# Adamtaranto/mimeo

Measured on NVIDIA B200. Metric: self-alignment Mbp/sec (genome Mbp annotated per second of hot-path time), higher is better.
Workload: dtype int32

## Files before the change

mimeo_b200/csrc/seed.cu:

```cuda
#include "primitives.cuh"
#include "seq.cuh"
#include "internal.cuh"
#include "xdrop_table.cuh"

namespace mb2 {

constexpr uint32_t KEY_INVALID = 1u << 24;
constexpr int S1_WINDOW = 30;
constexpr uint32_t S1_WINDOW_MASK = (1u << S1_WINDOW) - 1u;
constexpr int S1_RIGHT_WINDOWS = 2;
constexpr int S1_LEFT_WINDOWS = 3;
constexpr int S1_TAB = XT_SIZE;

__global__ void __launch_bounds__(256)
seed_keys_kernel(GenomeView T, uint32_t p_lo, uint32_t n, uint32_t* __restrict__ keys, uint32_t* __restrict__ pos) {
    const uint32_t k = blockIdx.x * blockDim.x + threadIdx.x;
    if (k >= n) return;
    const uint32_t p = p_lo + k;
    const uint32_t nw = nwindow32(T.sm, p) & SEED_WINDOW_MASK19;
    keys[k] = nw ? KEY_INVALID : seed_key(window32(T.pk, p));
    pos[k] = p;
}

__global__ void __launch_bounds__(256)
bucket_offsets_kernel(const uint32_t* __restrict__ keys, uint32_t n, uint32_t* __restrict__ off) {
    const uint32_t idx = blockIdx.x * blockDim.x + threadIdx.x;
    if (idx > n) return;
    const int64_t prev = idx == 0 ? -1 : (int64_t)keys[idx - 1];
    const int64_t cur = idx == n ? (int64_t)KEY_INVALID : (int64_t)min(keys[idx], KEY_INVALID);
    for (int64_t k = prev + 1; k <= cur; k++) off[k] = idx;
}

void build_seed_table(const Genome& T, uint32_t p_lo, uint32_t p_hi, SeedTable& tab) {
    const uint32_t n = p_hi - p_lo;
    ProfScope ps("seed_table_build");
    DevBuf<uint32_t> k0(n), k1(n), v0(n), v1(n);
    launch(seed_keys_kernel, cdiv(n, 256), 256, 0, view(T), p_lo, n, k0.get(), v0.get());
    const int w = radix_sort_bits<uint32_t, uint32_t>(k0.get(), k1.get(), v0.get(), v1.get(), n, 0, 25);
    tab.off.alloc((size_t)KEY_INVALID + 1);
    launch(bucket_offsets_kernel, cdiv((size_t)n + 1, 256), 256, 0, w ? k1.get() : k0.get(), n, tab.off.get());
    tab.pos = std::move(w ? v1 : v0);
    tab.p_lo = p_lo; tab.p_hi = p_hi;
}

constexpr int S1_DONE = 1 << 24;
constexpr int S1_D0 = 125;
constexpr int S1_MAX_XDROP = 8191 - 125 - 300;
__device__ __forceinline__ uint32_t s1_entry(uint32_t idx, int X) {
    const uint32_t q6 = idx >> 6, t6 = idx & 63;
    int sum = 0, mx = INT_MIN, mn = INT_MAX;
    for (int c = 0; c < 3; c++) {
        sum += sub_lut((((t6 >> (2 * c)) & 3u) << 2) | ((q6 >> (2 * c)) & 3u));
        mx = max(mx, sum); mn = min(mn, sum);
    }
    return ((uint32_t)sum << 22) | ((uint32_t)(mx + 125) << 13) | (uint32_t)(mn + X + 125);
}
__device__ __forceinline__ uint32_t s1_bits(uint32_t lo, uint32_t hi, int s) {
    return s <= 0 ? lo << (-s) : (s < 32 ? __funnelshift_r(lo, hi, s) : hi >> (s - 32));
}
template <uint32_t VOTES>
__device__ __forceinline__ void xdrop_window30(uint32_t tab_sa, uint32_t m10, uint32_t m9, uint64_t wt, uint64_t wq, uint32_t an, int X,
                                               int& best, int& D, uint32_t& nchunks) {
    int d_keep = 0;
    bool slow = false;
    if (D < S1_DONE / 2 && an) {
        int run = best - (D - 125);
        bool term = false;
        for (int c = 0; c < S1_WINDOW && !term; c++) {
            const int sc = (an & 1u) ? SCORE_N : sub_lut((uint32_t)((wt & 3) << 2 | (wq & 3)));
            wt >>= 2; wq >>= 2; an >>= 1;
            run += sc;
            if (run > best) best = run; else if (run < best - X) term = true;
        }
        nchunks += S1_WINDOW / 3;
        d_keep = term ? S1_DONE : (best - run) + 125;
        slow = true; D = S1_DONE;
    }
    const uint32_t tl = (uint32_t)wt, th = (uint32_t)(wt >> 32), ql = (uint32_t)wq, qh = (uint32_t)(wq >> 32);
    uint32_t parked = 0;
    int entered = S1_WINDOW / 3;
#pragma unroll
    for (int k = 0; k < S1_WINDOW / 3; k++) {
        if ((VOTES >> k) & 1u) { if (__all_sync(0xffffffffu, D >= S1_DONE / 2)) { entered = k; break; } }
        const uint32_t addr = ((s1_bits(tl, th, 6 * k - 2) & 0xFCu) | (s1_bits(ql, qh, 6 * k - 8) & 0x3F00u)) + tab_sa;
        uint32_t e;
        asm("ld.shared.u32 %0, [%1];" : "=r"(e) : "r"(addr));
        parked += (uint32_t)D;
        const bool term = (int)(e & 0x1FFFu) < D;
        const int dm = max(D, (int)__umulhi(e * m10, m9));
        best += dm - D;
        D = term ? S1_DONE : dm - __mulhi((int)e, (int)m10);
    }
    nchunks += (uint32_t)entered - (parked >> 24);
    if (slow) D = d_keep;
}
__device__ __forceinline__ uint32_t s1_pack(int best, int D) {
    return (uint32_t)best | ((D < S1_DONE / 2 ? (uint32_t)D : 0xFFFFu) << 16);
}
__device__ __forceinline__ void s1_unpack(uint32_t w, int& best, int& D) {
    best = (int)(w & 0xFFFFu);
    D = (w >> 16) == 0xFFFFu ? S1_DONE : (int)(w >> 16);
}

struct SeqBlock {
    uint64_t w[4];
    uint32_t n[4], s[4];
    uint32_t c0;
    __device__ __forceinline__ void windows(uint32_t p, uint64_t& f, uint64_t& l, uint64_t& r, uint32_t& fn, uint32_t& rn, uint32_t& ls) const {
        const uint32_t off = p - c0, sh = (off & 15u) * 2u;
        const bool b0 = off & 16u, b1 = off & 32u;
        uint32_t x[8], a[7], y[5];
#pragma unroll
        for (int m = 0; m < 4; m++) { x[2 * m] = (uint32_t)w[m]; x[2 * m + 1] = (uint32_t)(w[m] >> 32); }
#pragma unroll
        for (int m = 0; m < 7; m++) a[m] = b0 ? x[m + 1] : x[m];
#pragma unroll
        for (int m = 0; m < 5; m++) y[m] = b1 ? a[m + 2] : a[m];
        const uint32_t f0 = __funnelshift_r(y[0], y[1], sh), f1 = __funnelshift_r(y[1], y[2], sh);
        const uint32_t r0 = __funnelshift_r(y[2], y[3], sh), r1 = __funnelshift_r(y[3], y[4], sh);
        f = (uint64_t)f0 | ((uint64_t)f1 << 32); r = (uint64_t)r0 | ((uint64_t)r1 << 32);
        l = (uint64_t)__funnelshift_r(f0, f1, 24) | ((uint64_t)__funnelshift_r(f1, r0, 24) << 32);
        const uint32_t sn = off & 31u;
        const uint32_t n0 = b1 ? n[1] : n[0], n1 = b1 ? n[2] : n[1], n2 = b1 ? n[3] : n[2];
        fn = __funnelshift_r(n0, n1, sn); rn = __funnelshift_r(n1, n2, sn);
        const uint32_t s0 = b1 ? s[1] : s[0], s1 = b1 ? s[2] : s[1], s2 = b1 ? s[3] : s[2];
        ls = __funnelshift_r(__funnelshift_r(s0, s1, sn), __funnelshift_r(s1, s2, sn), 12);
    }
};
__device__ __forceinline__ SeqBlock load_block(const uint64_t* __restrict__ pk, const uint32_t* __restrict__ nm, const uint32_t* __restrict__ sm,
                                               uint32_t first) {
    SeqBlock b;
    b.c0 = first & ~63u;
    const uint32_t w0 = b.c0 >> 5;
    const uint4 a = *reinterpret_cast<const uint4*>(pk + w0), c = *reinterpret_cast<const uint4*>(pk + w0 + 2);
    b.w[0] = (uint64_t)a.x | ((uint64_t)a.y << 32); b.w[1] = (uint64_t)a.z | ((uint64_t)a.w << 32);
    b.w[2] = (uint64_t)c.x | ((uint64_t)c.y << 32); b.w[3] = (uint64_t)c.z | ((uint64_t)c.w << 32);
    const uint2 n0 = *reinterpret_cast<const uint2*>(nm + w0), n1 = *reinterpret_cast<const uint2*>(nm + w0 + 2);
    b.n[0] = n0.x; b.n[1] = n0.y; b.n[2] = n1.x; b.n[3] = n1.y;
    if (sm != nm) {
        const uint2 s0 = *reinterpret_cast<const uint2*>(sm + w0), s1 = *reinterpret_cast<const uint2*>(sm + w0 + 2);
        b.s[0] = s0.x; b.s[1] = s0.y; b.s[2] = s1.x; b.s[3] = s1.y;
    } else {
        b.s[0] = b.n[0]; b.s[1] = b.n[1]; b.s[2] = b.n[2]; b.s[3] = b.n[3];
    }
    return b;
}

__device__ __forceinline__ void append_survivors(bool survivor, uint32_t hi, uint32_t hj, uint32_t diag_bias, int lane,
                                                 uint64_t* __restrict__ surv, uint32_t surv_cap, unsigned long long* __restrict__ counters) {
    const uint32_t smask = __ballot_sync(0xffffffffu, survivor);
    if (smask) {
        unsigned long long basev = 0;
        if (lane == __ffs(smask) - 1) basev = atomicAdd(&counters[0], (unsigned long long)__popc(smask));
        basev = __shfl_sync(0xffffffffu, basev, __ffs(smask) - 1);
        if (survivor) {
            const unsigned long long slot = basev + __popc(smask & ((1u << lane) - 1u));
            if (slot < surv_cap) surv[slot] = ((uint64_t)(hi - hj + diag_bias) << 32) | hj;
        }
    }
}

constexpr int SC_NT = 256;
constexpr int SC_WARPS = SC_NT / 32;
constexpr int SC_NPROBE = 13;
constexpr int SC_HALF = 3;
constexpr int SC_STEPS = (SC_NPROBE + SC_HALF - 1) / SC_HALF;
constexpr int SC_RING = 128;
constexpr int SC_DQ = 64;

__device__ __forceinline__ void s1_later_window(const GenomeView& T, const GenomeView& Q, uint32_t hi, uint32_t hj, bool right, int b, int D,
                                                uint64_t& wt, uint64_t& wq, uint32_t& an) {
    wt = 0; wq = 0; an = 0;
    if (D >= S1_DONE / 2) return;
    if (right) {
        const uint32_t ct = hi + SEED_SPAN + S1_WINDOW * b, cq = hj + SEED_SPAN + S1_WINDOW * b;
        wt = window32(T.pk, ct); wq = window32(Q.pk, cq);
        an = (nwindow32(T.nm, ct) | nwindow32(Q.nm, cq)) & S1_WINDOW_MASK;
    } else {
        const uint32_t ct = hi + SEED_SPAN - S1_WINDOW * b - 32, cq = hj + SEED_SPAN - S1_WINDOW * b - 32;
        wt = rev2groups(window32(T.pk, ct)); wq = rev2groups(window32(Q.pk, cq));
        an = __brev(nwindow32(T.nm, ct) | nwindow32(Q.nm, cq)) & S1_WINDOW_MASK;
    }
}

template <int MINB, uint32_t TAILVOTES>
__global__ void __launch_bounds__(SC_NT, MINB)
seed_scan_kernel(GenomeView T, GenomeView Q, const uint32_t* __restrict__ off, const uint32_t* __restrict__ pos,
                 uint32_t q_lo, uint32_t q_n, int X, int K, int transition, uint32_t diag_bias,
                 uint64_t* __restrict__ surv, uint32_t surv_cap, unsigned long long* __restrict__ counters) {
    __shared__ uint32_t s1tab[S1_TAB];
    __shared__ uint32_t r_cum[SC_WARPS][SC_RING], r_b0[SC_WARPS][SC_RING], r_j[SC_WARPS][SC_RING];
    __shared__ uint4 r_defer[SC_WARPS][SC_DQ];
    __shared__ unsigned long long sh_stat[3];
    const int tid = threadIdx.x, lane = tid & 31, warp = tid >> 5;
    for (int e = tid; e < S1_TAB; e += SC_NT) s1tab[e] = s1_entry((uint32_t)e, X);
    const uint32_t s1tab_sa = (uint32_t)__cvta_generic_to_shared(s1tab);
    const uint32_t s1_m10 = q_n ? 1024u : 0u, s1_m9 = q_n ? 512u : 0u;
    if (tid < 3) sh_stat[tid] = 0;
    __syncthreads();
    uint32_t* __restrict__ rc = r_cum[warp];
    uint32_t* __restrict__ rb = r_b0[warp];
    uint32_t* __restrict__ rj = r_j[warp];
    uint4* __restrict__ dq = r_defer[warp];
    const int nprobe = transition ? SC_NPROBE : 1;
    const uint32_t nrounds = (q_n + 31) / 32;
    uint32_t round = 0;
    int part = SC_STEPS;
    bool exhausted = false;
    uint32_t head = 0, tail = 0;
    uint32_t cum_tail = 0, consumed = 0;
    uint32_t dq_head = 0, dq_tail = 0;
    unsigned long long n_lead = 0, n_cells = 0, n_hits = 0;
    for (;;) {
        while (cum_tail - consumed < 32u && !exhausted) {
            if (part == SC_STEPS) {
                unsigned long long r = 0;
                if (lane == 0) r = atomicAdd(&counters[CNT_WORK], 1ull);
                r = __shfl_sync(0xffffffffu, r, 0);
                if (r >= nrounds) { exhausted = true; break; }
                round = (uint32_t)r; part = 0;
            }
            const int p0 = part * SC_HALF, p1 = min(SC_NPROBE, p0 + SC_HALF);
            part++;
            const uint32_t jrel = round * 32 + lane;
            const uint32_t j = q_lo + jrel;
            const bool jvalid = jrel < q_n && (nwindow32(Q.sm, j) & SEED_WINDOW_MASK19) == 0;
            uint32_t key = 0;
            if (jvalid) key = seed_key(window32(Q.pk, j));
            uint32_t b0[SC_HALF], cnt[SC_HALF];
            uint32_t mine = 0, nne = 0;
#pragma unroll
            for (int q = 0; q < SC_HALF; q++) {
                const int pr = p0 + q;
                uint32_t c = 0, b = 0;
                if (jvalid && pr < p1 && pr < nprobe) {
                    const uint32_t kk = pr == 0 ? key : key ^ (2u << (2 * (pr - 1)));
                    b = off[kk];
                    c = off[kk + 1] - b;
                }
                b0[q] = b; cnt[q] = c;
                mine += c; nne += c ? 1u : 0u;
            }
            uint32_t sh = mine, sn = nne;
#pragma unroll
            for (int d = 1; d < 32; d <<= 1) {
                const uint32_t th = __shfl_up_sync(0xffffffffu, sh, d), tn = __shfl_up_sync(0xffffffffu, sn, d);
                if (lane >= d) { sh += th; sn += tn; }
            }
            const uint32_t tot_h = __shfl_sync(0xffffffffu, sh, 31), tot_n = __shfl_sync(0xffffffffu, sn, 31);
            uint32_t run = cum_tail + sh - mine, slot = tail + sn - nne;
#pragma unroll
            for (int q = 0; q < SC_HALF; q++) {
                if (cnt[q]) {
                    const uint32_t w = slot & (SC_RING - 1);
                    rc[w] = run; rb[w] = b0[q]; rj[w] = j;
                    run += cnt[q]; slot++;
                }
            }
            tail += tot_n; cum_tail += tot_h; n_hits += (lane == 0) ? tot_h : 0;
            __syncwarp();
        }
        const uint32_t pending = cum_tail - consumed, queued = dq_tail - dq_head;
        if (pending == 0 && queued == 0) break;
        uint32_t hi = 0, hj = 0, nchunks = 0;
        int best_r = 0, dr = S1_DONE, best_l = 0, dl = S1_DONE;
        bool live;
        if (queued >= 32u || pending == 0) {
            static_assert(S1_RIGHT_WINDOWS == 2 && S1_LEFT_WINDOWS == 3, "a batch runs right window 0 and left windows 0, 1; a drain the rest");
            const uint32_t nd = min(queued, 32u);
            live = (uint32_t)lane < nd;
            if (live) {
                const uint4 r = dq[(dq_head + (uint32_t)lane) & (SC_DQ - 1)];
                hi = r.x; hj = r.y;
                s1_unpack(r.z, best_r, dr);
                s1_unpack(r.w, best_l, dl);
            }
            dq_head += nd;
            uint64_t wt, wq; uint32_t an;
            if (!__all_sync(0xffffffffu, dr >= S1_DONE / 2)) {
                s1_later_window(T, Q, hi, hj, true, 1, dr, wt, wq, an);
                xdrop_window30<TAILVOTES>(s1tab_sa, s1_m10, s1_m9, wt, wq, an, X, best_r, dr, nchunks);
            }
            if (!__all_sync(0xffffffffu, dl >= S1_DONE / 2)) {
                s1_later_window(T, Q, hi, hj, false, 2, dl, wt, wq, an);
                xdrop_window30<TAILVOTES>(s1tab_sa, s1_m10, s1_m9, wt, wq, an, X, best_l, dl, nchunks);
            }
        } else {
            const uint32_t nb = min(pending, 32u);
            live = (uint32_t)lane < nb;
            const uint32_t h = consumed + (uint32_t)lane;
            uint32_t e_last = head;
            {
                const uint32_t di = head + (uint32_t)lane;
                const bool dv = (int32_t)(tail - di) > 0;
                const uint32_t ci = dv ? rc[di & (SC_RING - 1)] : 0u;
                const uint32_t first = ci - consumed;
                const uint32_t starts = __reduce_or_sync(0xffffffffu, (dv && lane > 0 && first < 32u) ? (1u << first) : 0u);
                if (live) {
                    const uint32_t lo = head + (uint32_t)__popc(starts & ((2u << lane) - 1u));
                    e_last = lo;
                    hi = pos[rb[lo & (SC_RING - 1)] + (h - rc[lo & (SC_RING - 1)])];
                    hj = rj[lo & (SC_RING - 1)];
                }
            }
            uint64_t lt = 0, lq = 0, rt = 0, rq = 0, ft = 0, fq = 0;
            uint32_t ln = 1, rn = 0, fn = 0;
            if (live) {
                const SeqBlock bt = load_block(T.pk, T.nm, T.sm, hi - 13), bq = load_block(Q.pk, Q.nm, Q.sm, hj - 13);
                uint32_t tfn, trn, tls, qfn, qrn, qls;
                bt.windows(hi - 13, ft, lt, rt, tfn, trn, tls);
                bq.windows(hj - 13, fq, lq, rq, qfn, qrn, qls);
                ln = (tls | qls) & SEED_WINDOW_MASK19;
                rn = (trn | qrn) & S1_WINDOW_MASK;
                fn = __brev(tfn | qfn) & S1_WINDOW_MASK;
                if (ln == 0 && seed_match(lt, lq, transition != 0)) live = false; else n_lead++;
            }
            if (live) { dr = S1_D0; dl = S1_D0; }
            xdrop_window30<0u>(s1tab_sa, s1_m10, s1_m9, rt, rq, rn, X, best_r, dr, nchunks);
            xdrop_window30<0u>(s1tab_sa, s1_m10, s1_m9, rev2groups(ft), rev2groups(fq), fn, X, best_l, dl, nchunks);
            if (!__all_sync(0xffffffffu, dl >= S1_DONE / 2)) {
                uint64_t wt, wq; uint32_t an;
                s1_later_window(T, Q, hi, hj, false, 1, dl, wt, wq, an);
                xdrop_window30<TAILVOTES>(s1tab_sa, s1_m10, s1_m9, wt, wq, an, X, best_l, dl, nchunks);
            }
            const bool defer = live && (dr < S1_DONE / 2 || dl < S1_DONE / 2);
            const uint32_t dmask = __ballot_sync(0xffffffffu, defer);
            if (defer) {
                dq[(dq_tail + (uint32_t)__popc(dmask & ((1u << lane) - 1u))) & (SC_DQ - 1)] =
                    make_uint4(hi, hj, s1_pack(best_r, dr), s1_pack(best_l, dl));
                live = false;
            }
            dq_tail += (uint32_t)__popc(dmask);
            consumed += nb;
            uint32_t e = __shfl_sync(0xffffffffu, e_last, (int)nb - 1);
            const uint32_t next_cum = (e + 1 < tail) ? rc[(e + 1) & (SC_RING - 1)] : cum_tail;
            head = ((int32_t)(next_cum - consumed) > 0) ? e : e + 1;
        }
        n_cells += 3ull * nchunks;
        append_survivors(live && (dr < S1_DONE / 2 || dl < S1_DONE / 2 || best_r + best_l >= K), hi, hj, diag_bias, lane, surv, surv_cap, counters);
        __syncwarp();
    }
    if (n_lead) atomicAdd(&sh_stat[1], n_lead);
    if (n_cells) atomicAdd(&sh_stat[2], n_cells);
    if (n_hits) atomicAdd(&sh_stat[0], n_hits);
    __syncthreads();
    if (tid < 3 && sh_stat[tid]) atomicAdd(&counters[1 + tid], sh_stat[tid]);
}

void seed_scan(const Genome& T, const Genome& Q, const SeedTable& tab, uint32_t q_lo, uint32_t q_hi, const AlignParams& p,
               uint64_t* surv, uint32_t surv_cap, unsigned long long* counters) {
    const uint32_t n = q_hi - q_lo;
    if (n == 0) return;
    MB2_REQUIRE(p.xdrop >= XT_MIN_XDROP, -2, "x-drop below 251 is not supported by the three-column extension table");
    MB2_REQUIRE(p.xdrop <= S1_MAX_XDROP, -2, "x-drop above 7766 is not supported by the first-stage extension table");
    ProfScope ps("seed_scan");
    const unsigned nrounds = cdiv(n, 32);
    static const int minb = getenv("MB2_SCAN_MINB") ? atoi(getenv("MB2_SCAN_MINB")) : 4;
    auto go = [&](auto kern) {
        int per_sm = 0;
        MB2_CUDA(cudaOccupancyMaxActiveBlocksPerMultiprocessor(&per_sm, kern, SC_NT, 0));
        const unsigned grid = std::min<unsigned>(cdiv(nrounds, SC_WARPS), (unsigned)ctx().sm_count * (unsigned)std::max(1, per_sm));
        launch(kern, grid, SC_NT, 0, view(T), view(Q), tab.off.get(), tab.pos.get(), q_lo, n, p.xdrop,
               p.hspthresh, p.transition, (uint32_t)Q.G, surv, surv_cap, counters);
    };
    if (minb <= 3) go(seed_scan_kernel<3, 0x148u>); else go(seed_scan_kernel<4, 0x148u>);
}

}
```

Baseline: 460.9.

## Extend seed block load to cover second left x-drop window from registers

The per-seed sequence block now loads one extra leading 64-bit packed word and N-mask word. This lets the second left-extension window be extracted by funnel shifts from registers instead of issuing separate global window loads in s1_later_window. The kernel's launch bounds are also replaced with explicit __maxnreg__ caps (56 or 80) to control register pressure from the larger block. It adds an unconditional extra load per live seed, even when the second left window is never needed, and reads at w0-1, which may fall before the buffer start near position zero.

```diff
diff --git a/mimeo_b200/csrc/seed.cu b/mimeo_b200/csrc/seed.cu
--- a/mimeo_b200/csrc/seed.cu
+++ b/mimeo_b200/csrc/seed.cu
@@ -103,26 +103,30 @@
 }
 
 struct SeqBlock {
-    uint64_t w[4];
-    uint32_t n[4], s[4];
+    uint64_t w[5];
+    uint32_t n[5], s[4];
     uint32_t c0;
-    __device__ __forceinline__ void windows(uint32_t p, uint64_t& f, uint64_t& l, uint64_t& r, uint32_t& fn, uint32_t& rn, uint32_t& ls) const {
+    __device__ __forceinline__ void windows(uint32_t p, uint64_t& f, uint64_t& g, uint64_t& l, uint64_t& r,
+                                            uint32_t& fn, uint32_t& gn, uint32_t& rn, uint32_t& ls) const {
         const uint32_t off = p - c0, sh = (off & 15u) * 2u;
         const bool b0 = off & 16u, b1 = off & 32u;
-        uint32_t x[8], a[7], y[5];
-#pragma unroll
-        for (int m = 0; m < 4; m++) { x[2 * m] = (uint32_t)w[m]; x[2 * m + 1] = (uint32_t)(w[m] >> 32); }
-#pragma unroll
-        for (int m = 0; m < 7; m++) a[m] = b0 ? x[m + 1] : x[m];
-#pragma unroll
-        for (int m = 0; m < 5; m++) y[m] = b1 ? a[m + 2] : a[m];
-        const uint32_t f0 = __funnelshift_r(y[0], y[1], sh), f1 = __funnelshift_r(y[1], y[2], sh);
-        const uint32_t r0 = __funnelshift_r(y[2], y[3], sh), r1 = __funnelshift_r(y[3], y[4], sh);
+        uint32_t x[10], a[9], y[7];
+#pragma unroll
+        for (int m = 0; m < 5; m++) { x[2 * m] = (uint32_t)w[m]; x[2 * m + 1] = (uint32_t)(w[m] >> 32); }
+#pragma unroll
+        for (int m = 0; m < 9; m++) a[m] = b0 ? x[m + 1] : x[m];
+#pragma unroll
+        for (int m = 0; m < 7; m++) y[m] = b1 ? a[m + 2] : a[m];
+        const uint32_t e0 = __funnelshift_r(y[0], y[1], sh), e1 = __funnelshift_r(y[1], y[2], sh);
+        const uint32_t f0 = __funnelshift_r(y[2], y[3], sh), f1 = __funnelshift_r(y[3], y[4], sh);
+        const uint32_t r0 = __funnelshift_r(y[4], y[5], sh), r1 = __funnelshift_r(y[5], y[6], sh);
         f = (uint64_t)f0 | ((uint64_t)f1 << 32); r = (uint64_t)r0 | ((uint64_t)r1 << 32);
+        g = (uint64_t)__funnelshift_r(e0, e1, 4) | ((uint64_t)__funnelshift_r(e1, f0, 4) << 32);
         l = (uint64_t)__funnelshift_r(f0, f1, 24) | ((uint64_t)__funnelshift_r(f1, r0, 24) << 32);
         const uint32_t sn = off & 31u;
-        const uint32_t n0 = b1 ? n[1] : n[0], n1 = b1 ? n[2] : n[1], n2 = b1 ? n[3] : n[2];
+        const uint32_t nl = b1 ? n[1] : n[0], n0 = b1 ? n[2] : n[1], n1 = b1 ? n[3] : n[2], n2 = b1 ? n[4] : n[3];
         fn = __funnelshift_r(n0, n1, sn); rn = __funnelshift_r(n1, n2, sn);
+        gn = __funnelshift_r(__funnelshift_r(nl, n0, sn), fn, 2);
         const uint32_t s0 = b1 ? s[1] : s[0], s1 = b1 ? s[2] : s[1], s2 = b1 ? s[3] : s[2];
         ls = __funnelshift_r(__funnelshift_r(s0, s1, sn), __funnelshift_r(s1, s2, sn), 12);
     }
@@ -133,15 +137,17 @@
     b.c0 = first & ~63u;
     const uint32_t w0 = b.c0 >> 5;
     const uint4 a = *reinterpret_cast<const uint4*>(pk + w0), c = *reinterpret_cast<const uint4*>(pk + w0 + 2);
-    b.w[0] = (uint64_t)a.x | ((uint64_t)a.y << 32); b.w[1] = (uint64_t)a.z | ((uint64_t)a.w << 32);
-    b.w[2] = (uint64_t)c.x | ((uint64_t)c.y << 32); b.w[3] = (uint64_t)c.z | ((uint64_t)c.w << 32);
+    b.w[0] = pk[w0 - 1];
+    b.w[1] = (uint64_t)a.x | ((uint64_t)a.y << 32); b.w[2] = (uint64_t)a.z | ((uint64_t)a.w << 32);
+    b.w[3] = (uint64_t)c.x | ((uint64_t)c.y << 32); b.w[4] = (uint64_t)c.z | ((uint64_t)c.w << 32);
     const uint2 n0 = *reinterpret_cast<const uint2*>(nm + w0), n1 = *reinterpret_cast<const uint2*>(nm + w0 + 2);
-    b.n[0] = n0.x; b.n[1] = n0.y; b.n[2] = n1.x; b.n[3] = n1.y;
+    b.n[0] = nm[w0 - 1];
+    b.n[1] = n0.x; b.n[2] = n0.y; b.n[3] = n1.x; b.n[4] = n1.y;
     if (sm != nm) {
         const uint2 s0 = *reinterpret_cast<const uint2*>(sm + w0), s1 = *reinterpret_cast<const uint2*>(sm + w0 + 2);
         b.s[0] = s0.x; b.s[1] = s0.y; b.s[2] = s1.x; b.s[3] = s1.y;
     } else {
-        b.s[0] = b.n[0]; b.s[1] = b.n[1]; b.s[2] = b.n[2]; b.s[3] = b.n[3];
+        b.s[0] = b.n[1]; b.s[1] = b.n[2]; b.s[2] = b.n[3]; b.s[3] = b.n[4];
     }
     return b;
 }
@@ -184,7 +190,7 @@
 }
 
 template <int MINB, uint32_t TAILVOTES>
-__global__ void __launch_bounds__(SC_NT, MINB)
+__global__ void __maxnreg__(MINB >= 4 ? 56 : 80)
 seed_scan_kernel(GenomeView T, GenomeView Q, const uint32_t* __restrict__ off, const uint32_t* __restrict__ pos,
                  uint32_t q_lo, uint32_t q_n, int X, int K, int transition, uint32_t diag_bias,
                  uint64_t* __restrict__ surv, uint32_t surv_cap, unsigned long long* __restrict__ counters) {
@@ -303,26 +309,24 @@
                     hj = rj[lo & (SC_RING - 1)];
                 }
             }
-            uint64_t lt = 0, lq = 0, rt = 0, rq = 0, ft = 0, fq = 0;
-            uint32_t ln = 1, rn = 0, fn = 0;
+            uint64_t lt = 0, lq = 0, rt = 0, rq = 0, ft = 0, fq = 0, gt = 0, gq = 0;
+            uint32_t ln = 1, rn = 0, fn = 0, gn = 0;
             if (live) {
                 const SeqBlock bt = load_block(T.pk, T.nm, T.sm, hi - 13), bq = load_block(Q.pk, Q.nm, Q.sm, hj - 13);
-                uint32_t tfn, trn, tls, qfn, qrn, qls;
-                bt.windows(hi - 13, ft, lt, rt, tfn, trn, tls);
-                bq.windows(hj - 13, fq, lq, rq, qfn, qrn, qls);
+                uint32_t tfn, tgn, trn, tls, qfn, qgn, qrn, qls;
+                bt.windows(hi - 13, ft, gt, lt, rt, tfn, tgn, trn, tls);
+                bq.windows(hj - 13, fq, gq, lq, rq, qfn, qgn, qrn, qls);
                 ln = (tls | qls) & SEED_WINDOW_MASK19;
                 rn = (trn | qrn) & S1_WINDOW_MASK;
                 fn = __brev(tfn | qfn) & S1_WINDOW_MASK;
+                gn = __brev(tgn | qgn) & S1_WINDOW_MASK;
                 if (ln == 0 && seed_match(lt, lq, transition != 0)) live = false; else n_lead++;
             }
             if (live) { dr = S1_D0; dl = S1_D0; }
             xdrop_window30<0u>(s1tab_sa, s1_m10, s1_m9, rt, rq, rn, X, best_r, dr, nchunks);
             xdrop_window30<0u>(s1tab_sa, s1_m10, s1_m9, rev2groups(ft), rev2groups(fq), fn, X, best_l, dl, nchunks);
-            if (!__all_sync(0xffffffffu, dl >= S1_DONE / 2)) {
-                uint64_t wt, wq; uint32_t an;
-                s1_later_window(T, Q, hi, hj, false, 1, dl, wt, wq, an);
-                xdrop_window30<TAILVOTES>(s1tab_sa, s1_m10, s1_m9, wt, wq, an, X, best_l, dl, nchunks);
-            }
+            if (!__all_sync(0xffffffffu, dl >= S1_DONE / 2))
+                xdrop_window30<TAILVOTES>(s1tab_sa, s1_m10, s1_m9, rev2groups(gt), rev2groups(gq), gn, X, best_l, dl, nchunks);
             const bool defer = live && (dr < S1_DONE / 2 || dl < S1_DONE / 2);
             const uint32_t dmask = __ballot_sync(0xffffffffu, defer);
             if (defer) {
```

After: 474.3, median of 6. 2.9% higher.
